# ihh/dnastore

Hardware: NVIDIA B200
Metric: viterbi_dp_cells_per_sec (higher is better)
Workload: dtype f64

## Files before the change

### dnastore_b200/csrc/viterbi_fill_batch.cu

```cuda
#include <cuda_runtime.h>

#include <cstdint>

#include "viterbi_batch.h"
#include "viterbi_kernels.h"

namespace dnab {
namespace {

__device__ __forceinline__ uint32_t smemAddr(const void* p) { return (uint32_t)__cvta_generic_to_shared(p); }
__device__ __forceinline__ double negInf() { return __longlong_as_double(0xFFF0000000000000LL); }
__device__ __forceinline__ double dmax(double a, double b) { return (a < b) ? b : a; }

__device__ __forceinline__ double2 ldsRow(uint32_t a) {
  double2 v;
  asm volatile("ld.volatile.shared.v2.f64 {%0,%1}, [%2];" : "=d"(v.x), "=d"(v.y) : "r"(a));
  return v;
}
__device__ __forceinline__ void stsRow(uint32_t a, double s, double d) {
  asm volatile("st.volatile.shared.v2.f64 [%0], {%1,%2};" ::"r"(a), "d"(s), "d"(d) : "memory");
}
__device__ __forceinline__ double2 ldPub2(const double2* p) {
  double2 v;
  asm volatile("ld.relaxed.gpu.global.v2.f64 {%0,%1}, [%2];" : "=d"(v.x), "=d"(v.y) : "l"(p) : "memory");
  return v;
}
__device__ __forceinline__ void stPub2(double2* p, double s, double d) {
  asm volatile("st.relaxed.gpu.global.v2.f64 [%0], {%1,%2};" ::"l"(p), "d"(s), "d"(d) : "memory");
}
__device__ __forceinline__ void stRecord(uint8_t* p, uint32_t v) {
  asm volatile("st.global.cs.u8 [%0], %1;" ::"l"(p), "r"(v) : "memory");
}
__device__ __forceinline__ uint32_t ldVolatileGlobal32(const uint32_t* p) {
  uint32_t v;
  asm volatile("ld.relaxed.gpu.global.u32 %0, [%1];" : "=r"(v) : "l"(p) : "memory");
  return v;
}
__device__ __forceinline__ unsigned long long ldAcquire64(const unsigned long long* p) {
  unsigned long long v;
  asm volatile("ld.acquire.gpu.global.u64 %0, [%1];" : "=l"(v) : "l"(p) : "memory");
  return v;
}

enum : uint32_t { kCtlFlag = 0, kCtlWake = 4, kCtlDecision = 8, kCtlPending = 16, kCtlPhase = 17, kCtlLock = 18, kCtlSeen = 32 };
constexpr uint32_t kKeepRecord = 0x100u;
constexpr uint32_t kKeepRecordWide = 0x10000u;

__device__ __forceinline__ void fenceRelease() { asm volatile("fence.release.gpu;" ::: "memory"); }
__device__ __forceinline__ void stRecordEarly(uint8_t* p, uint32_t v) { asm volatile("st.global.u8 [%0], %1;" ::"l"(p), "r"(v) : "memory"); }
__device__ __forceinline__ unsigned long long policyEvictLast() {
  unsigned long long pol;
  asm volatile("createpolicy.fractional.L2::evict_last.b64 %0, 1.0;" : "=l"(pol));
  return pol;
}
__device__ __forceinline__ double ldCarried(const double* p, unsigned long long pol) {
  double v;
  asm volatile("ld.global.L2::cache_hint.f64 %0, [%1], %2;" : "=d"(v) : "l"(p), "l"(pol) : "memory");
  return v;
}
__device__ __forceinline__ void stCarried(double* p, double v, unsigned long long pol) {
  asm volatile("st.global.L2::cache_hint.f64 [%0], %1, %2;" ::"l"(p), "d"(v), "l"(pol) : "memory");
}
__device__ __forceinline__ void redAdd32(uint32_t* p, uint32_t v) {
  asm volatile("red.relaxed.gpu.global.add.u32 [%0], %1;" ::"l"(p), "r"(v) : "memory");
}
__device__ __forceinline__ void stRelaxed32(uint32_t* p, uint32_t v) {
  asm volatile("st.relaxed.gpu.global.u32 [%0], %1;" ::"l"(p), "r"(v) : "memory");
}

}

template <int W, int KMAX, bool kTeam, bool kDebug, bool kWide>
__global__ void __launch_bounds__(W * 32, 1)
    viterbiFillBatchKernel(const __grid_constant__ BatchTables tb, const __grid_constant__ BatchArgs args) {
  extern __shared__ __align__(16) unsigned char smem[];
  constexpr uint32_t nThreads = W * 32;
  const uint32_t tid = threadIdx.x, lane = tid & 31u, warp = tid >> 5, lane16 = lane * 16u;
  const uint32_t T = kTeam ? tb.T : 1u, M = tb.M, k = tb.k, Np = T * M, N = tb.nStates, K2 = k + 2;
  const uint32_t team = kTeam ? blockIdx.x / T : blockIdx.x, rank = kTeam ? blockIdx.x - team * T : 0u;
  const uint32_t nSlots = (M + W - 1) / W;
  const double NEG = negInf();
  const BatchLayout lay = makeBatchLayout(M, tb.maxIn, tb.maxOut, tb.nSyms, kTeam);
  auto wideCounts = [&](const uint4& h) { return __ldg(tb.wide + bhWideNo(h)); };
  auto nOutLocalOf = [&](const uint4& h) { return (kWide && bhWide(h)) ? (wideCounts(h).w & 0xFFFFu) : bhNOutLocal(h); };
  auto nOutOf = [&](const uint4& h) { return (kWide && bhWide(h)) ? (wideCounts(h).w >> 16) : bhNOut(h); };

  const uint32_t aSD = smemAddr(smem + lay.sd);
  uint32_t* maskCur = reinterpret_cast<uint32_t*>(smem + lay.maskA);
  uint32_t* maskNext = reinterpret_cast<uint32_t*>(smem + lay.maskB);
  uint32_t* remInS = reinterpret_cast<uint32_t*>(smem + lay.remIn);
  uint32_t* clsOffS = reinterpret_cast<uint32_t*>(smem + lay.cls);
  uint32_t* clsStS = clsOffS + kNotifyClasses + 1;
  uint4* hdrS = reinterpret_cast<uint4*>(smem + lay.hdr);
  uint2* hdr2S = reinterpret_cast<uint2*>(smem + lay.hdr2);
  uint2* inS = reinterpret_cast<uint2*>(smem + lay.inE);
  uint2* relS = reinterpret_cast<uint2*>(smem + lay.relE);
  uint32_t* outS = reinterpret_cast<uint32_t*>(smem + lay.outE);
  double* tsE = reinterpret_cast<double*>(smem + lay.tsE);
  double* subS = reinterpret_cast<double*>(smem + lay.sub);
  volatile uint32_t* ctl = reinterpret_cast<volatile uint32_t*>(smem + lay.ctl);

  {
    for (uint32_t i = tid; i < M; i += nThreads) {
      hdrS[i] = tb.hdr[rank * M + i];
      hdr2S[i] = tb.hdr2[rank * M + i];
      if (kTeam) {
        remInS[i] = tb.remoteIn[rank * M + i];
        clsStS[i] = tb.clsStates[rank * M + i];
      }
      maskCur[i] = 0;
      maskNext[i] = 0;
    }
    const uint32_t inBase = tb.rankInOff[rank], nIn = tb.rankInOff[rank + 1] - inBase;
    for (uint32_t i = tid; i < nIn; i += nThreads) {
      uint2 e = tb.inEdges[inBase + i];
      if (!beRemote(e)) e.x = aSD + (e.x - rank * M) * 512u;
      inS[i] = e;
      uint2 q = tb.relEdges[inBase + i];
      relS[i] = q;
    }
    __syncthreads();
    for (uint32_t i = tid; i < M; i += nThreads) {
      const uint2 h2 = hdr2S[i];
      uint32_t nLoc = (h2.y & 0xFFu) + ((h2.y >> 8) & 0xFFu);
      if (kWide && bhWide(hdrS[i])) {
        const uint32_t lc = wideCounts(hdrS[i]).y;
        nLoc = (lc & 0xFFFFu) + (lc >> 16);
      }
      for (uint32_t j = 0; j < nLoc; ++j) relS[h2.x + j].x = aSD + (relS[h2.x + j].x - rank * M) * 512u;
    }
    const uint32_t outBase = tb.rankOutOff[rank], nOut = tb.rankOutOff[rank + 1] - outBase;
    for (uint32_t i = tid; i < nOut; i += nThreads) outS[i] = tb.outEdges[outBase + i];
    for (uint32_t i = tid; i < tb.nSyms * 16; i += nThreads) tsE[i] = tb.tsE[i];
    if (tid < 16) subS[tid] = tb.sub[tid];
    if (tid < 64) ctl[tid] = 0;
    if (kTeam && tid <= kNotifyClasses) clsOffS[tid] = tb.clsOff[rank * (kNotifyClasses + 1) + tid];
  }
  __syncthreads();

  const uint32_t privKinds = 2 + k;
  double* const privT = args.priv + (size_t)team * Np * privKinds * 32 + lane;
  const unsigned long long polLast = policyEvictLast();
  double2* const sdPubT = args.sdPub + (size_t)team * 2 * Np * 32;
  uint32_t* const notifyT = args.teamState + (size_t)team * T * kNotifyClasses;
  uint32_t* const passiveT = args.teamPassive + (size_t)team * 2;
  uint32_t notifySeen = 0;
  unsigned long long* const bar = args.barrier + team;
  unsigned long long barTarget = 0;
  uint32_t col = 0;

  auto teamBarrier = [&]() {
    __syncthreads();
    if (!kTeam) return;
    barTarget += T;
    if (tid == 0) {
      fenceRelease();
      atomicAdd(bar, 1ull);
      while (ldAcquire64(bar) < barTarget) {
      }
    }
    __syncthreads();
  };

  unsigned long long dbgLevels = 0, dbgVisits = 0, dbgEdges = 0, dbgWakes = 0, dbgClosure = 0, dbgRecord = 0, dbgPassive = 0, dbgInit = 0, dbgBarrier = 0, dbgRelaxCyc = 0, dbgFlushCyc = 0;

  for (int64_t group = team; group < args.nGroups; group += args.nTeams) {
    const int64_t slotIdx = group * 32 + lane;
    int64_t r = -1;
    if (args.order)
      r = args.order[slotIdx];
    else if (args.readBase + slotIdx < args.nReads)
      r = args.readBase + slotIdx;
    const int32_t L = r >= 0 ? args.readLen[r] : -1;
    const uint8_t* seq = r >= 0 ? args.packed + args.byteOff[r] : nullptr;
    int32_t Lmax = L;
    for (int sh = 16; sh > 0; sh >>= 1) Lmax = max(Lmax, __shfl_xor_sync(0xFFFFFFFFu, Lmax, sh));
    uint8_t* const predG = args.pred + (size_t)group * (size_t)(args.maxLen + 1) * N * K2 * 32;
    uint8_t* const predWideG = kWide ? args.predWide + (size_t)group * (size_t)(args.maxLen + 1) * tb.nWide * 64 + lane : nullptr;
    unsigned long long win = 0;
    uint32_t xNext = 0;

    for (int32_t pos = 0; pos <= Lmax; ++pos) {
      const bool act = pos <= L;
      if (pos < L) {
        if ((pos & 31) == 0) win = *reinterpret_cast<const unsigned long long*>(seq + (size_t)(pos >> 5) * 8);
        xNext = (uint32_t)(win >> (2 * (pos & 31))) & 3u;
      }
      const uint32_t par = col & 1u;
      ++col;
      unsigned long long stamp = 0;
      if (kDebug) stamp = clock64();
      double2* const sdPubCol = sdPubT + (size_t)par * Np * 32;
      double2* const sdPubNext = sdPubT + (size_t)(par ^ 1u) * Np * 32;
      uint32_t* const passiveCol = passiveT + par;

#pragma unroll 4
      for (uint32_t sl = 0; sl < nSlots; ++sl) {
        const uint32_t d = sl * W + warp;
        if (d < M) {
          double s0;
          if (pos == 0) {
            const uint4 h = hdrS[d];
            s0 = (!bhPad(h) && (tb.local || (rank == tb.startRank && d == tb.startLocal))) ? 0.0 : NEG;
            if (kTeam && bhRemoteOut(h)) stPub2(sdPubCol + (size_t)(rank * M + d) * 32 + lane, s0, NEG);
          } else
            s0 = ldCarried(privT + (size_t)(rank * M + d) * privKinds * 32, polLast);
          stsRow(aSD + d * 512u + lane16, s0, NEG);
        }
      }
      if (tid < 8) ctl[tid] = 0;
      if (tid == 0) {
        ctl[kCtlPending] = 0u;
        ctl[kCtlPhase] = 0u;
      }
      if (kDebug) {
        const unsigned long long t = clock64();
        dbgInit += t - stamp;
        stamp = t;
      }
      teamBarrier();
      if (kTeam && rank == 0 && tid == 0) stRelaxed32(passiveT + (par ^ 1u), 0u);
      if (kDebug) {
        const unsigned long long t = clock64();
        dbgBarrier += t - stamp;
        stamp = t;
      }

      const bool asyncClosure = args.asyncClosure != 0;
      uint32_t* const idleS = const_cast<uint32_t*>(reinterpret_cast<volatile uint32_t*>(ctl) + kCtlPending);
      uint32_t* const lockS = const_cast<uint32_t*>(reinterpret_cast<volatile uint32_t*>(ctl) + kCtlLock);
      uint32_t remotePending = 0;
      auto relax = [&](uint32_t sl, uint32_t m, bool allIn) -> bool {
        const uint32_t d = sl * W + warp;
        const uint4 h = hdrS[d];
        const uint2 h2 = hdr2S[d];
        uint32_t nLE = h2.y & 0xFFu, nLN = (h2.y >> 8) & 0xFFu, nRE = (h2.y >> 16) & 0xFFu, nRN = h2.y >> 24;
        if (kWide && bhWide(h)) {
          const uint4 wc = wideCounts(h);
          nLE = wc.y & 0xFFFFu;
          nLN = wc.y >> 16;
          nRE = wc.z & 0xFFFFu;
          nRN = wc.z >> 16;
        }
        const uint32_t eLN = nLE + nLN, eRE = eLN + nRE, nIn = eRE + nRN;
        const uint2* const rel = relS + h2.x;
        const uint32_t aOwn = aSD + d * 512u + lane16;
        const double2 own = ldsRow(aOwn);
        double s = own.x, dd = own.y;
        const char* const scoreBase = reinterpret_cast<const char*>(tb.symScore);
        auto scoreOf = [&](const uint2& e) { return *reinterpret_cast<const double*>(scoreBase + e.y); };
        auto emitFrom = [&](const double2 v, const uint2& e) {
          dd = dmax(dd, dmax(v.y + tb.delExtend, v.x + tb.delOpen) + scoreOf(e));
          if (kDebug) ++dbgEdges;
        };
        auto nullFrom = [&](const double2 v, const uint2& e) {
          const double sc = scoreOf(e);
          dd = dmax(dd, v.y + sc);
          s = dmax(s, v.x + sc);
          if (kDebug) ++dbgEdges;
        };
        auto one = [&](uint32_t j) {
          const uint2 e = rel[j];
          if (j < eLN) {
            const double2 v = ldsRow(e.x + lane16);
            if (j < nLE)
              emitFrom(v, e);
            else
              nullFrom(v, e);
          } else if (kTeam) {
            const double2 v = ldPub2(sdPubCol + (size_t)e.x * 32 + lane);
            if (j < eRE)
              emitFrom(v, e);
            else
              nullFrom(v, e);
          }
        };
        if (allIn || nIn <= 4u) {
          uint32_t j = 0;
#pragma unroll 1
          for (; j < nLE; ++j) {
            const uint2 e = rel[j];
            emitFrom(ldsRow(e.x + lane16), e);
          }
#pragma unroll 1
          for (; j < eLN; ++j) {
            const uint2 e = rel[j];
            nullFrom(ldsRow(e.x + lane16), e);
          }
          if (kTeam) {
#pragma unroll 1
            for (; j < eRE; ++j) {
              const uint2 e = rel[j];
              emitFrom(ldPub2(sdPubCol + (size_t)e.x * 32 + lane), e);
            }
#pragma unroll 1
            for (; j < nIn; ++j) {
              const uint2 e = rel[j];
              nullFrom(ldPub2(sdPubCol + (size_t)e.x * 32 + lane), e);
            }
          }
        } else {
          while (m) {
            const uint32_t j = (uint32_t)__ffs((int)m) - 1u;
            m &= m - 1u;
            if (j == 31u)
              for (uint32_t jj = 31; jj < nIn; ++jj) one(jj);
            else
              one(j);
          }
        }
        s = dmax(s, dd + tb.delEnd);
        const bool grew = act && ((s > own.x) || (dd > own.y));
        if (!__any_sync(0xFFFFFFFFu, grew)) return false;
        stsRow(aOwn, s, dd);
        if (kTeam && bhRemoteOut(h)) {
          stPub2(sdPubCol + (size_t)(rank * M + d) * 32 + lane, s, dd);
          remotePending |= 1u << sl;
        }
        const uint32_t nLoc = nOutLocalOf(h), outOff = bhOutOff(h);
        uint32_t* const flagTo = asyncClosure ? maskCur : maskNext;
#pragma unroll 1
        for (uint32_t o = lane; o < nLoc; o += 32) {
          const uint32_t w = outS[outOff + o];
          atomicOr(flagTo + boLocal(w), 1u << boBit(w));
        }
        return true;
      };
      auto flushRemote = [&]() {
        if (!kTeam || !remotePending) return;
        uint32_t nNotes = 0;
        for (uint32_t rp = remotePending; rp; rp &= rp - 1u) {
          const uint4 h = hdrS[((uint32_t)__ffs((int)rp) - 1u) * W + warp];
          nNotes += nOutOf(h) - nOutLocalOf(h);
        }
        const bool eager = args.eagerNotify != 0;
        if (lane == 0) redAdd32(passiveCol, 0u - (eager ? 2u * nNotes : nNotes));
        if (eager) {
          __syncwarp();
          for (uint32_t rp = remotePending; rp; rp &= rp - 1u) {
            const uint4 h = hdrS[((uint32_t)__ffs((int)rp) - 1u) * W + warp];
            const uint32_t first = bhOutOff(h) + nOutLocalOf(h), last = bhOutOff(h) + nOutOf(h);
            for (uint32_t o = first + lane; o < last; o += 32) redAdd32(notifyT + outS[o], 1u);
          }
        }
        fenceRelease();
        __syncwarp();
        while (remotePending) {
          const uint32_t sl = (uint32_t)__ffs((int)remotePending) - 1u;
          remotePending &= remotePending - 1u;
          const uint4 h = hdrS[sl * W + warp];
          const uint32_t first = bhOutOff(h) + nOutLocalOf(h), last = bhOutOff(h) + nOutOf(h);
          for (uint32_t o = first + lane; o < last; o += 32) redAdd32(notifyT + outS[o], 1u);
        }
      };

      if (asyncClosure) {
        const uint32_t iMine = lane * W + warp;
        const bool mineValid = lane < nSlots && iMine < M;
        bool idle = false;
        for (uint32_t sl = 0; sl < nSlots; ++sl) {
          const uint32_t d = sl * W + warp;
          if (d >= M) break;
          if (lane == 0) maskCur[d] = 0u;
          __syncwarp();
          unsigned long long tr = 0;
          if (kDebug) tr = clock64();
          relax(sl, 0, true);
          if (kDebug) dbgRelaxCyc += clock64() - tr;
        }
        {
          unsigned long long tr = 0;
          if (kDebug) tr = clock64();
          flushRemote();
          if (kDebug) dbgFlushCyc += clock64() - tr;
        }
        for (;;) {
          uint32_t mym = 0;
          if (mineValid) mym = reinterpret_cast<volatile uint32_t*>(maskCur)[iMine];
          uint32_t work = __ballot_sync(0xFFFFFFFFu, mym != 0);
          if (work) {
            if (idle) {
              if (lane == 0) atomicSub(idleS, 1u);
              idle = false;
              __syncwarp();
            }
            if (mym) atomicAnd(maskCur + iMine, ~mym);
            while (work) {
              const uint32_t sl = (uint32_t)__ffs((int)work) - 1u;
              work &= work - 1u;
              const uint32_t m = __shfl_sync(0xFFFFFFFFu, mym, sl);
              if (kDebug) ++dbgVisits;
              unsigned long long tr = 0;
              if (kDebug) tr = clock64();
              relax(sl, m, false);
              if (kDebug) dbgRelaxCyc += clock64() - tr;
            }
            {
              unsigned long long tr = 0;
              if (kDebug) tr = clock64();
              flushRemote();
              if (kDebug) dbgFlushCyc += clock64() - tr;
            }
            continue;
          }
          if (!idle) {
            if (lane == 0) atomicAdd(idleS, 1u);
            idle = true;
          }
          if (ctl[kCtlPhase] != 0u) break;
          uint32_t mine = 0;
          if (lane == 0) mine = ctl[kCtlLock] == 0u && atomicCAS(lockS, 0u, 1u) == 0u;
          if (!__shfl_sync(0xFFFFFFFFu, mine, 0)) {
            if (args.idleNs) __nanosleep(args.idleNs);
            continue;
          }
          auto unlock = [&]() {
            __syncwarp();
            if (lane == 0) {
              __threadfence_block();
              atomicExch(lockS, 0u);
            }
          };
          if (ctl[kCtlPhase] != 0u) {
            unlock();
            break;
          }
          bool quiet = false;
          if (ctl[kCtlPending] == W) {
            bool any = false;
            for (uint32_t i = lane; i < M; i += 32) any |= reinterpret_cast<volatile uint32_t*>(maskCur)[i] != 0u;
            quiet = !__any_sync(0xFFFFFFFFu, any) && ctl[kCtlPending] == W;
          }
          uint32_t action = 0;
          uint32_t delta = 0;
          if (!kTeam) {
            if (quiet) action = 2;
          } else {
            uint32_t seen = ctl[kCtlSeen + lane];
            auto pollClasses = [&]() -> uint32_t {
              const uint32_t c = ldVolatileGlobal32(notifyT + rank * kNotifyClasses + lane);
              delta = c - seen;
              seen = c;
              return __any_sync(0xFFFFFFFFu, delta != 0u) ? __reduce_add_sync(0xFFFFFFFFu, delta) : 0u;
            };
            uint32_t tot = pollClasses();
            if (tot) {
              if (lane == 0) redAdd32(passiveCol, tot);
              action = 1;
            } else if (quiet) {
              unsigned long long t0 = 0;
              if (kDebug) t0 = clock64();
              if (lane == 0) redAdd32(passiveCol, 1u);
              for (;;) {
                tot = pollClasses();
                if (tot) {
                  if (lane == 0) redAdd32(passiveCol, tot - 1u);
                  action = 1;
                  break;
                }
                uint32_t p = lane == 0 ? ldVolatileGlobal32(passiveCol) : 0u;
                p = __shfl_sync(0xFFFFFFFFu, p, 0);
                if (p == T) {
                  action = 2;
                  break;
                }
              }
              if (kDebug) dbgPassive += clock64() - t0;
            }
            ctl[kCtlSeen + lane] = seen;
          }
          if (action == 2) {
            if (lane == 0) ctl[kCtlPhase] = 1u;
            unlock();
          } else if (action == 1) {
            if (kDebug) ++dbgWakes;
            if (lane == 0) atomicSub(idleS, 1u);
            idle = false;
            __syncwarp();
            for (uint32_t notified = __ballot_sync(0xFFFFFFFFu, delta != 0u); notified; notified &= notified - 1u) {
              const uint32_t c = (uint32_t)__ffs((int)notified) - 1u;
              for (uint32_t q = clsOffS[c] + lane; q < clsOffS[c + 1]; q += 32) {
                const uint32_t i = clsStS[q];
                atomicOr(maskCur + i, remInS[i]);
              }
            }
            unlock();
          } else {
            unlock();
            if (args.idleNs) __nanosleep(args.idleNs / 2);
          }
        }
        __syncthreads();
      } else
      {
        auto notifyTotal = [&]() -> uint32_t {
          uint32_t t = 0;
          for (uint32_t q = 0; q < kNotifyClasses; ++q) t += ldVolatileGlobal32(notifyT + rank * kNotifyClasses + q);
          return t;
        };
        uint32_t lvl = 0;
        bool activated = false;
        for (uint32_t sl = 0; sl < nSlots; ++sl)
          if (sl * W + warp < M) activated |= relax(sl, 0, true);
        flushRemote();
        for (;;) {
          if (activated && lane == 0) ctl[kCtlFlag + ((lvl + 1) & 3u)] = 1u;
          if (tid == 0) {
            ctl[kCtlFlag + ((lvl + 2) & 3u)] = 0u;
            ctl[kCtlWake + ((lvl + 2) & 3u)] = 0u;
          }
          __syncthreads();
          {
            uint32_t* t = maskCur;
            maskCur = maskNext;
            maskNext = t;
          }
          ++lvl;
          const bool haveLocal = ctl[kCtlFlag + (lvl & 3u)] != 0;
          bool wake = kTeam && ctl[kCtlWake + (lvl & 3u)] != 0;
          if (!haveLocal && !wake) {
            if (!kTeam) break;
            if (tid == 0) {
              unsigned long long t0 = 0;
              if (kDebug) t0 = clock64();
              uint32_t decision;
              redAdd32(passiveCol, 1u);
              for (;;) {
                const uint32_t c = notifyTotal();
                if (c != notifySeen) {
                  redAdd32(passiveCol, c - notifySeen - 1u);
                  notifySeen = c;
                  decision = 1;
                  break;
                }
                if (ldVolatileGlobal32(passiveCol) == T) {
                  decision = 2;
                  break;
                }
              }
              ctl[kCtlDecision] = decision;
              if (kDebug) dbgPassive += clock64() - t0;
            }
            __syncthreads();
            if (ctl[kCtlDecision] == 2u) break;
            wake = true;
          }
          if (kDebug && haveLocal) ++dbgLevels;
          if (kDebug && wake) ++dbgWakes;
          activated = false;
          uint32_t st = 0;
          if (kTeam && tid == 0) st = notifyTotal();
          const uint32_t iMine = lane * W + warp;
          uint32_t mym = 0;
          if (lane < nSlots && iMine < M) {
            if (haveLocal) {
              mym = maskCur[iMine];
              if (mym) maskCur[iMine] = 0;
            }
            if (wake) mym |= remInS[iMine];
          }
          uint32_t work = __ballot_sync(0xFFFFFFFFu, mym != 0);
          while (work) {
            const uint32_t sl = (uint32_t)__ffs((int)work) - 1u;
            work &= work - 1u;
            const uint32_t m = __shfl_sync(0xFFFFFFFFu, mym, sl);
            if (kDebug) ++dbgVisits;
            activated |= relax(sl, m, false);
          }
          flushRemote();
          if (kTeam && tid == 0 && st != notifySeen) {
            redAdd32(passiveCol, st - notifySeen);
            notifySeen = st;
            ctl[kCtlWake + ((lvl + 1) & 3u)] = 1u;
          }
        }
      }
      if (kDebug) {
        const unsigned long long t = clock64();
        dbgClosure += t - stamp;
        stamp = t;
      }

      {
        double bv = NEG;
        uint32_t bo = 0xFFFFFFFFu;
        double pfB = NEG, pfT[KMAX];
        auto fetch = [&](uint32_t sl) {
          const uint32_t d = sl * W + warp;
          if (d < M && pos > 0) {
            const double* row = privT + (size_t)(rank * M + d) * privKinds * 32;
            pfB = ldCarried(row + 32, polLast);
#pragma unroll
            for (uint32_t t = 0; t < (uint32_t)KMAX; ++t)
              if (t < k) pfT[t] = ldCarried(row + 64 + 32 * t, polLast);
          }
        };
#pragma unroll
        for (uint32_t t = 0; t < (uint32_t)KMAX; ++t) pfT[t] = NEG;
        fetch(0);
        for (uint32_t sl = 0; sl < nSlots; ++sl) {
          const uint32_t d = sl * W + warp;
          if (d >= M) break;
          const double curB = pfB;
          double curT[KMAX];
#pragma unroll
          for (uint32_t t = 0; t < (uint32_t)KMAX; ++t) curT[t] = pfT[t];
          if (sl + 1 < nSlots) fetch(sl + 1);
          const uint4 h = hdrS[d];
          if (bhPad(h)) continue;
          const bool wide = kWide && bhWide(h);
          uint32_t nE = bhNEmit(h), nIn = nE + bhNNull(h);
          if (wide) {
            const uint32_t c = wideCounts(h).x;
            nE = c & 0xFFFFu;
            nIn = nE + (c >> 16);
          }
          const uint32_t inOff = bhInOff(h), mdl = bhMdl(h), orig = h.w;
          constexpr uint32_t keep = kWide ? kKeepRecordWide : kKeepRecord;
          const uint32_t none = wide ? kWideNoPred : kNoPred;
          double* const row = privT + (size_t)(rank * M + d) * privKinds * 32;
          const double2 own = ldsRow(aSD + d * 512u + lane16);
          const double sH = own.x, dH = own.y;
          double best = pos > 0 ? curB : NEG, bestD = NEG, s0n = NEG, bEn = NEG;
          uint32_t idx = pos > 0 ? keep : none, idxD = none, idxEn = none;
          uint32_t j = 0;
#pragma unroll 1
          for (; j < nE; ++j) {
            const uint2 e = inS[inOff + j];
            const uint32_t sym = beSym(e);
            const double2 v = (kTeam && beRemote(e)) ? ldPub2(sdPubCol + (size_t)e.x * 32 + lane) : ldsRow(e.x + lane16);
            double c = v.y + tb.tsDext[sym];
            if (c > bestD) {
              bestD = c;
              idxD = 2 * j;
            }
            c = v.x + tb.tsDopen[sym];
            if (c > bestD) {
              bestD = c;
              idxD = 2 * j + 1;
            }
            const uint32_t b4 = beBase(e) * 4 + xNext;
            s0n = dmax(s0n, ((v.x + tb.symScore[sym]) + tb.noGap) + subS[b4]);
            c = v.x + tsE[sym * 16 + b4];
            if (c > bEn) {
              bEn = c;
              idxEn = j;
            }
          }
#pragma unroll 1
          for (; j < nIn; ++j) {
            const uint2 e = inS[inOff + j];
            const double2 v = (kTeam && beRemote(e)) ? ldPub2(sdPubCol + (size_t)e.x * 32 + lane) : ldsRow(e.x + lane16);
            const double sc = tb.symScore[beSym(e)];
            double c = v.x + sc;
            if (c > best) {
              best = c;
              idx = j;
            }
            c = v.y + sc;
            if (c > bestD) {
              bestD = c;
              idxD = nE + j;
            }
          }
          {
            const double c = dH + tb.delEnd;
            if (c > best) {
              best = c;
              idx = nIn;
            }
          }
          if (mdl > 0 && pos > 0) {
            const double parked = curT[0];
            if (parked > best) {
              best = parked;
              idx = nIn + 1;
            }
          }
          if (tb.local && pos == 0) {
            const double2 v0 = (kTeam && tb.startRank != rank)
                                   ? ldPub2(sdPubCol + (size_t)(tb.startRank * M + tb.startLocal) * 32 + lane)
                                   : ldsRow(aSD + tb.startLocal * 512u + lane16);
            if (v0.x + 0.0 > best) {
              best = v0.x + 0.0;
              idx = nIn + 2;
            }
          }
          uint8_t* const pr = predG + ((size_t)pos * N + orig) * K2 * 32 + lane;
          uint8_t* const prW = wide ? predWideG + ((size_t)pos * tb.nWide + bhWideNo(h)) * 64 : nullptr;
          if (act) {
            if (idx != keep) stRecord(pr, idx);
            stRecord(pr + 32, idxD);
            if (wide) {
              if (idx != keep) stRecord(prW, idx >> 8);
              stRecord(prW + 32, idxD >> 8);
            }
          }
          double tNow[KMAX];
#pragma unroll
          for (uint32_t t = 0; t < (uint32_t)KMAX; ++t) {
            tNow[t] = NEG;
            if (t < k) {
              uint32_t idxT = kNoPred;
              if (pos > 0 && t < mdl) {
                double shifted = NEG;
                if (t + 1 < (uint32_t)KMAX && t + 1 < mdl) shifted = curT[t + 1 < (uint32_t)KMAX ? t + 1 : 0];
                if (shifted > NEG) idxT = 0;
                if (sH + tb.tsT[t] > shifted) idxT = 1;
                tNow[t] = dmax(shifted, (sH + tb.tanDup) + tb.len[t]);
              }
              if (act) stRecord(pr + (2 + t) * 32, idxT);
            }
          }
          if (kDebug && args.cells && group == 0 && lane == 0 && act) {
            double* cell = args.cells + ((size_t)pos * N + orig) * K2;
            cell[0] = sH;
            cell[1] = dH;
#pragma unroll
            for (uint32_t t = 0; t < (uint32_t)KMAX; ++t)
              if (t < k) cell[2 + t] = tNow[t];
          }
          if (mdl > 0) {
#pragma unroll
            for (uint32_t t = 0; t < (uint32_t)KMAX; ++t)
              if (t < mdl) {
                const double v = tNow[t] + subS[bhCtx(h, t) * 4 + xNext];
                if (t == 0) s0n = dmax(s0n, v);
                stCarried(row + 64 + 32 * t, v, polLast);
              }
          }
          stCarried(row, s0n, polLast);
          stCarried(row + 32, bEn, polLast);
          if (pos < L) {
            stRecordEarly(pr + (size_t)N * K2 * 32, idxEn);
            if (wide) stRecordEarly(prW + (size_t)tb.nWide * 64, idxEn >> 8);
          }
          if (kTeam && bhRemoteOut(h)) stPub2(sdPubNext + (size_t)(rank * M + d) * 32 + lane, s0n, NEG);
          if (!tb.local) {
            if (rank == tb.endRank && d == tb.endLocal && pos == L && r >= 0) args.loglike[r] = sH;
          } else if (sH > bv || (sH == bv && orig < bo)) {
            bv = sH;
            bo = orig;
          }
        }
        if (tb.local && pos == L) {
          args.partVal[((size_t)group * T * W + rank * W + warp) * 32 + lane] = bv;
          args.partOrig[((size_t)group * T * W + rank * W + warp) * 32 + lane] = bo;
        }
      }
      __syncthreads();
      if (kDebug) dbgRecord += clock64() - stamp;
    }
  }
  if (kDebug && args.dbg && lane == 0 && rank == 0) {
    if (warp == 0) atomicAdd(&args.dbg[1], dbgLevels);
    atomicAdd(&args.dbg[2], dbgVisits);
    atomicAdd(&args.dbg[3], dbgEdges);
    if (warp == 0) atomicAdd(&args.dbg[4], dbgClosure);
    if (warp == 0) atomicAdd(&args.dbg[5], dbgRecord);
    atomicAdd(&args.dbg[6], dbgWakes);
    atomicAdd(&args.dbg[7], dbgPassive);
    if (warp == 0) atomicAdd(&args.dbg[8], dbgInit);
    if (warp == 0) atomicAdd(&args.dbg[9], dbgBarrier);
    atomicAdd(&args.dbg[10], dbgRelaxCyc);
    atomicAdd(&args.dbg[11], dbgFlushCyc);
  }
}

__global__ void viterbiTracebackBatchKernel(const BatchTraceTables tb, const BatchTraceArgs args) {
  const int64_t slot = (int64_t)blockIdx.x * blockDim.x + threadIdx.x;
  if (slot >= args.nSlots) return;
  int64_t read = -1;
  if (args.order)
    read = args.order[slot];
  else if (args.readBase + slot < args.nReads)
    read = args.readBase + slot;
  if (read < 0) return;
  const int64_t group = slot >> 5;
  const uint32_t lane = (uint32_t)(slot & 31);
  const uint32_t N = tb.nStates, k = tb.k, K2 = k + 2;
  const int32_t L = args.readLen[read];
  const double NEG = negInf();

  uint32_t state;
  double ll;
  if (!tb.local) {
    state = N - 1;
    ll = args.loglike[read];
  } else {
    double bv = NEG;
    uint32_t bo = 0xFFFFFFFFu;
    for (uint32_t r = 0; r < tb.T; ++r) {
      const double v = args.partVal[((size_t)group * tb.T + r) * 32 + lane];
      const uint32_t o = args.partOrig[((size_t)group * tb.T + r) * 32 + lane];
      if (o == 0xFFFFFFFFu) continue;
      if (v > bv || (v == bv && o < bo)) {
        bv = v;
        bo = o;
      }
    }
    state = bo == 0xFFFFFFFFu ? 0u : bo;
    ll = bv;
    args.loglike[read] = ll;
  }

  char* out = args.decoded + (size_t)read * args.decodedStride;
  int32_t* path = args.path ? args.path + (size_t)read * 3 * args.pathStride : nullptr;
  int32_t nOut = 0, nPath = 0;
  int32_t status = DNAB_READ_OK_;
  if (!(ll > NEG)) {
    args.decodedLen[read] = 0;
    args.status[read] = DNAB_READ_NO_DECODING_;
    if (args.pathLen) args.pathLen[read] = 0;
    return;
  }
  const uint8_t* predG = args.pred + (size_t)group * (size_t)(args.maxLen + 1) * N * K2 * 32 + lane;
  const uint8_t* predWideG = args.predWide + (size_t)group * (size_t)(args.maxLen + 1) * tb.nWide * 64 + lane;
  int32_t pos = L;
  uint32_t mut = 0;
  const int32_t cap = args.decodedStride;
  while (pos >= 0 && state != 0) {
    if (path) {
      if (nPath < args.pathStride) {
        path[3 * nPath] = (int32_t)state;
        path[3 * nPath + 1] = pos;
        path[3 * nPath + 2] = (int32_t)mut;
      } else
        status = DNAB_READ_OVERFLOW_;
    }
    ++nPath;
    uint32_t p = predG[(((size_t)pos * N + state) * K2 + mut) * 32];
    uint32_t none = kNoPred;
    if (tb.wideOf && mut < 2) {
      const uint32_t wn = tb.wideOf[state];
      if (wn != 0xFFFFFFFFu) {
        p |= (uint32_t)predWideG[(((size_t)pos * tb.nWide + wn) * 2 + mut) * 32] << 8;
        none = kWideNoPred;
      }
    }
    if (p == none) {
      status = DNAB_READ_TRACEBACK_FAILED_;
      break;
    }
    const uint32_t e0 = tb.emitOff[state], nE = tb.emitOff[state + 1] - e0;
    const uint32_t n0 = tb.nullOff[state], nIn = nE + (tb.nullOff[state + 1] - n0);
    uint32_t sym = 0;
    if (mut == 0) {
      if (p < nE) {
        sym = tb.emitSym[e0 + p];
        state = tb.emitSrc[e0 + p];
        --pos;
      } else if (p < nIn) {
        sym = tb.nullSym[n0 + (p - nE)];
        state = tb.nullSrc[n0 + (p - nE)];
      } else if (p == nIn) {
        mut = 1;
      } else if (p == nIn + 1) {
        mut = 2;
        --pos;
      } else {
        state = 0;
      }
    } else if (mut == 1) {
      if (p < 2 * nE) {
        sym = tb.emitSym[e0 + (p >> 1)];
        state = tb.emitSrc[e0 + (p >> 1)];
        mut = (p & 1) ? 0 : 1;
      } else {
        sym = tb.nullSym[n0 + (p - 2 * nE)];
        state = tb.nullSrc[n0 + (p - 2 * nE)];
      }
    } else {
      if (p == 0) {
        mut += 1;
        --pos;
      } else
        mut = 0;
    }
    if (sym) {
      if (nOut < cap)
        out[cap - 1 - nOut] = (char)tb.symChar[sym];
      else
        status = DNAB_READ_OVERFLOW_;
      ++nOut;
    }
  }
  const int32_t kept = nOut < cap ? nOut : cap;
  for (int32_t i = 0; i < kept; ++i) out[i] = out[cap - kept + i];
  args.decodedLen[read] = kept;
  args.status[read] = status;
  if (args.pathLen) args.pathLen[read] = nPath;
}

typedef void (*BatchKernelPtr)(const BatchTables, const BatchArgs);
template <int W, int KMAX, bool kWide>
static BatchKernelPtr pickBatchKernelWK(bool team, bool debug) {
  if (debug) return team ? viterbiFillBatchKernel<W, KMAX, true, true, kWide> : viterbiFillBatchKernel<W, KMAX, false, true, kWide>;
  return team ? viterbiFillBatchKernel<W, KMAX, true, false, kWide> : viterbiFillBatchKernel<W, KMAX, false, false, kWide>;
}
static uint32_t batchWarps(uint32_t warps) { return warps > 24 ? 32u : warps > 16 ? 24u : 16u; }
template <bool kWide>
static BatchKernelPtr pickBatchKernelW(const BatchTables& tb, uint32_t warps, bool debug) {
  const bool team = tb.T > 1;
  const uint32_t w = batchWarps(warps);
  if (w == 32) return tb.k <= 2 ? pickBatchKernelWK<32, 2, kWide>(team, debug) : pickBatchKernelWK<32, kMaxK, kWide>(team, debug);
  if (w == 24) return tb.k <= 2 ? pickBatchKernelWK<24, 2, kWide>(team, debug) : pickBatchKernelWK<24, kMaxK, kWide>(team, debug);
  return tb.k <= 2 ? pickBatchKernelWK<16, 2, kWide>(team, debug) : pickBatchKernelWK<16, kMaxK, kWide>(team, debug);
}
static BatchKernelPtr pickBatchKernel(const BatchTables& tb, uint32_t warps, bool debug) {
  return tb.nWide ? pickBatchKernelW<true>(tb, warps, debug) : pickBatchKernelW<false>(tb, warps, debug);
}

cudaError_t queryBatchTeams(const BatchTables& tb, uint32_t warps, uint32_t smemBytes, int* ctasPerSm) {
  BatchKernelPtr kern = pickBatchKernel(tb, warps, false);
  cudaError_t err = cudaFuncSetAttribute(kern, cudaFuncAttributeMaxDynamicSharedMemorySize, (int)smemBytes);
  if (err != cudaSuccess) return err;
  return cudaOccupancyMaxActiveBlocksPerMultiprocessor(ctasPerSm, kern, (int)(batchWarps(warps) * 32), smemBytes);
}

cudaError_t launchFillBatch(const BatchTables& tb, const BatchArgs& args, uint32_t warps, uint32_t smemBytes,
                            cudaStream_t stream, size_t persistBytes) {
  const bool debug = args.dbg != nullptr || args.cells != nullptr;
  BatchKernelPtr kern = pickBatchKernel(tb, warps, debug);
  cudaError_t err = cudaFuncSetAttribute(kern, cudaFuncAttributeMaxDynamicSharedMemorySize, (int)smemBytes);
  if (err != cudaSuccess) return err;
  cudaLaunchConfig_t cfg{};
  cfg.gridDim = dim3(args.nTeams * tb.T);
  cfg.blockDim = dim3(batchWarps(warps) * 32);
  cfg.dynamicSmemBytes = smemBytes;
  cfg.stream = stream;
  cudaLaunchAttribute attr[2];
  unsigned nAttr = 0;
  if (tb.T > 1) {
    attr[nAttr].id = cudaLaunchAttributeCooperative;
    attr[nAttr].val.cooperative = 1;
    ++nAttr;
  }
  if (persistBytes) {
    attr[nAttr].id = cudaLaunchAttributeAccessPolicyWindow;
    attr[nAttr].val.accessPolicyWindow.base_ptr = args.priv;
    attr[nAttr].val.accessPolicyWindow.num_bytes = persistBytes;
    attr[nAttr].val.accessPolicyWindow.hitRatio = 1.0f;
    attr[nAttr].val.accessPolicyWindow.hitProp = cudaAccessPropertyPersisting;
    attr[nAttr].val.accessPolicyWindow.missProp = cudaAccessPropertyStreaming;
    ++nAttr;
  }
  cfg.attrs = attr;
  cfg.numAttrs = nAttr;
  return cudaLaunchKernelEx(&cfg, kern, tb, args);
}

cudaError_t launchTracebackBatch(const BatchTraceTables& tb, const BatchTraceArgs& args, cudaStream_t stream) {
  const int threads = 64;
  const int blocks = (int)((args.nSlots + threads - 1) / threads);
  viterbiTracebackBatchKernel<<<blocks, threads, 0, stream>>>(tb, args);
  return cudaGetLastError();
}

}
```

Measured before the change: 50.64 billion.

## Batch edge gathers in closure relax and prefetch next slot's predecessor rows

The closure relax step now handles incoming edges in groups of four. It loads all edge descriptors, scores and source rows before doing any max updates, so the load latencies overlap instead of being serialized. The final recurrence pass software-pipelines the first four incoming edges and their source rows for the next slot while the current slot computes. This adds register pressure and branchy bookkeeping for the mask and tail handling. The prefetch may also read shared or published rows before later relaxations update them, which needs care around ordering.

```diff
diff --git a/dnastore_b200/csrc/viterbi_fill_batch.cu b/dnastore_b200/csrc/viterbi_fill_batch.cu
--- a/dnastore_b200/csrc/viterbi_fill_batch.cu
+++ b/dnastore_b200/csrc/viterbi_fill_batch.cu
@@ -45,6 +45,7 @@
 enum : uint32_t { kCtlFlag = 0, kCtlWake = 4, kCtlDecision = 8, kCtlPending = 16, kCtlPhase = 17, kCtlLock = 18, kCtlSeen = 32 };
 constexpr uint32_t kKeepRecord = 0x100u;
 constexpr uint32_t kKeepRecordWide = 0x10000u;
+constexpr uint32_t kGather = 4;
 
 __device__ __forceinline__ void fenceRelease() { asm volatile("fence.release.gpu;" ::: "memory"); }
 __device__ __forceinline__ void stRecordEarly(uint8_t* p, uint32_t v) { asm volatile("st.global.u8 [%0], %1;" ::"l"(p), "r"(v) : "memory"); }
@@ -248,65 +249,66 @@
         const double2 own = ldsRow(aOwn);
         double s = own.x, dd = own.y;
         const char* const scoreBase = reinterpret_cast<const char*>(tb.symScore);
-        auto scoreOf = [&](const uint2& e) { return *reinterpret_cast<const double*>(scoreBase + e.y); };
-        auto emitFrom = [&](const double2 v, const uint2& e) {
-          dd = dmax(dd, dmax(v.y + tb.delExtend, v.x + tb.delOpen) + scoreOf(e));
+        auto emitFrom = [&](const double2 v, const double sc) {
+          dd = dmax(dd, dmax(v.y + tb.delExtend, v.x + tb.delOpen) + sc);
           if (kDebug) ++dbgEdges;
         };
-        auto nullFrom = [&](const double2 v, const uint2& e) {
-          const double sc = scoreOf(e);
+        auto nullFrom = [&](const double2 v, const double sc) {
           dd = dmax(dd, v.y + sc);
           s = dmax(s, v.x + sc);
           if (kDebug) ++dbgEdges;
         };
-        auto one = [&](uint32_t j) {
-          const uint2 e = rel[j];
-          if (j < eLN) {
-            const double2 v = ldsRow(e.x + lane16);
-            if (j < nLE)
-              emitFrom(v, e);
-            else
-              nullFrom(v, e);
-          } else if (kTeam) {
-            const double2 v = ldPub2(sdPubCol + (size_t)e.x * 32 + lane);
-            if (j < eRE)
-              emitFrom(v, e);
-            else
-              nullFrom(v, e);
-          }
+        auto gather = [&](const uint32_t(&js)[kGather], uint32_t n) {
+          uint2 e[kGather];
+          double sc[kGather];
+          double2 v[kGather];
+#pragma unroll
+          for (uint32_t i = 0; i < kGather; ++i) {
+            e[i] = make_uint2(0u, 0u);
+            sc[i] = 0.0;
+            v[i] = make_double2(0.0, 0.0);
+            if (i < n) e[i] = rel[js[i]];
+          }
+#pragma unroll
+          for (uint32_t i = 0; i < kGather; ++i)
+            if (i < n) {
+              sc[i] = *reinterpret_cast<const double*>(scoreBase + e[i].y);
+              v[i] = (!kTeam || js[i] < eLN) ? ldsRow(e[i].x + lane16) : ldPub2(sdPubCol + (size_t)e[i].x * 32 + lane);
+            }
+#pragma unroll
+          for (uint32_t i = 0; i < kGather; ++i)
+            if (i < n) {
+              if (js[i] < nLE || (kTeam && js[i] >= eLN && js[i] < eRE))
+                emitFrom(v[i], sc[i]);
+              else
+                nullFrom(v[i], sc[i]);
+            }
         };
-        if (allIn || nIn <= 4u) {
-          uint32_t j = 0;
-#pragma unroll 1
-          for (; j < nLE; ++j) {
-            const uint2 e = rel[j];
-            emitFrom(ldsRow(e.x + lane16), e);
-          }
-#pragma unroll 1
-          for (; j < eLN; ++j) {
-            const uint2 e = rel[j];
-            nullFrom(ldsRow(e.x + lane16), e);
-          }
-          if (kTeam) {
-#pragma unroll 1
-            for (; j < eRE; ++j) {
-              const uint2 e = rel[j];
-              emitFrom(ldPub2(sdPubCol + (size_t)e.x * 32 + lane), e);
-            }
-#pragma unroll 1
-            for (; j < nIn; ++j) {
-              const uint2 e = rel[j];
-              nullFrom(ldPub2(sdPubCol + (size_t)e.x * 32 + lane), e);
-            }
-          }
+        if (nIn <= kGather) {
+          uint32_t all[kGather];
+#pragma unroll
+          for (uint32_t i = 0; i < kGather; ++i) all[i] = i;
+          gather(all, nIn);
         } else {
-          while (m) {
-            const uint32_t j = (uint32_t)__ffs((int)m) - 1u;
-            m &= m - 1u;
-            if (j == 31u)
-              for (uint32_t jj = 31; jj < nIn; ++jj) one(jj);
-            else
-              one(j);
+          uint32_t mm = allIn ? (nIn >= 32u ? 0xFFFFFFFFu : (1u << nIn) - 1u) : m, tail = 31;
+          while (mm) {
+            uint32_t js[kGather], n = 0;
+#pragma unroll
+            for (uint32_t i = 0; i < kGather; ++i) {
+              js[i] = 0;
+              if (mm) {
+                const uint32_t j = (uint32_t)__ffs((int)mm) - 1u;
+                if (j < 31u) {
+                  js[i] = j;
+                  mm &= mm - 1u;
+                } else {
+                  js[i] = tail++;
+                  if (tail >= nIn) mm = 0;
+                }
+                n = i + 1;
+              }
+            }
+            gather(js, n);
           }
         }
         s = dmax(s, dd + tb.delEnd);
@@ -585,19 +587,51 @@
         double bv = NEG;
         uint32_t bo = 0xFFFFFFFFu;
         double pfB = NEG, pfT[KMAX];
+        uint32_t pfIn = 0;
+        uint2 pfE[kGather];
+        double2 pfV[kGather];
+#pragma unroll
+        for (uint32_t i = 0; i < kGather; ++i) {
+          pfE[i] = make_uint2(0u, 0u);
+          pfV[i] = make_double2(NEG, NEG);
+        }
+        auto srcRow = [&](const uint2& e) {
+          return (kTeam && beRemote(e)) ? ldPub2(sdPubCol + (size_t)e.x * 32 + lane) : ldsRow(e.x + lane16);
+        };
+        auto inCounts = [&](const uint4& h, uint32_t& nE, uint32_t& nIn) {
+          nE = bhNEmit(h);
+          nIn = nE + bhNNull(h);
+          if (kWide && bhWide(h)) {
+            const uint32_t c = wideCounts(h).x;
+            nE = c & 0xFFFFu;
+            nIn = nE + (c >> 16);
+          }
+        };
         auto fetch = [&](uint32_t sl) {
           const uint32_t d = sl * W + warp;
-          if (d < M && pos > 0) {
-            const double* row = privT + (size_t)(rank * M + d) * privKinds * 32;
-            pfB = ldCarried(row + 32, polLast);
-#pragma unroll
-            for (uint32_t t = 0; t < (uint32_t)KMAX; ++t)
-              if (t < k) pfT[t] = ldCarried(row + 64 + 32 * t, polLast);
+          pfIn = 0;
+          if (d < M) {
+            if (pos > 0) {
+              const double* row = privT + (size_t)(rank * M + d) * privKinds * 32;
+              pfB = ldCarried(row + 32, polLast);
+#pragma unroll
+              for (uint32_t t = 0; t < (uint32_t)KMAX; ++t)
+                if (t < k) pfT[t] = ldCarried(row + 64 + 32 * t, polLast);
+            }
+            const uint4 h = hdrS[d];
+            uint32_t nE;
+            inCounts(h, nE, pfIn);
+#pragma unroll
+            for (uint32_t i = 0; i < kGather; ++i)
+              if (i < pfIn) pfE[i] = inS[bhInOff(h) + i];
           }
         };
 #pragma unroll
         for (uint32_t t = 0; t < (uint32_t)KMAX; ++t) pfT[t] = NEG;
         fetch(0);
+#pragma unroll
+        for (uint32_t i = 0; i < kGather; ++i)
+          if (i < pfIn) pfV[i] = srcRow(pfE[i]);
         for (uint32_t sl = 0; sl < nSlots; ++sl) {
           const uint32_t d = sl * W + warp;
           if (d >= M) break;
@@ -605,16 +639,27 @@
           double curT[KMAX];
 #pragma unroll
           for (uint32_t t = 0; t < (uint32_t)KMAX; ++t) curT[t] = pfT[t];
-          if (sl + 1 < nSlots) fetch(sl + 1);
+          uint2 curE[kGather];
+          double2 curV[kGather];
+#pragma unroll
+          for (uint32_t i = 0; i < kGather; ++i) {
+            curE[i] = pfE[i];
+            curV[i] = pfV[i];
+          }
+          if (sl + 1 < nSlots)
+            fetch(sl + 1);
+          else
+            pfIn = 0;
           const uint4 h = hdrS[d];
-          if (bhPad(h)) continue;
+          if (bhPad(h)) {
+#pragma unroll
+            for (uint32_t i = 0; i < kGather; ++i)
+              if (i < pfIn) pfV[i] = srcRow(pfE[i]);
+            continue;
+          }
           const bool wide = kWide && bhWide(h);
-          uint32_t nE = bhNEmit(h), nIn = nE + bhNNull(h);
-          if (wide) {
-            const uint32_t c = wideCounts(h).x;
-            nE = c & 0xFFFFu;
-            nIn = nE + (c >> 16);
-          }
+          uint32_t nE, nIn;
+          inCounts(h, nE, nIn);
           const uint32_t inOff = bhInOff(h), mdl = bhMdl(h), orig = h.w;
           constexpr uint32_t keep = kWide ? kKeepRecordWide : kKeepRecord;
           const uint32_t none = wide ? kWideNoPred : kNoPred;
@@ -623,12 +668,8 @@
           const double sH = own.x, dH = own.y;
           double best = pos > 0 ? curB : NEG, bestD = NEG, s0n = NEG, bEn = NEG;
           uint32_t idx = pos > 0 ? keep : none, idxD = none, idxEn = none;
-          uint32_t j = 0;
-#pragma unroll 1
-          for (; j < nE; ++j) {
-            const uint2 e = inS[inOff + j];
+          auto emitCand = [&](const uint2& e, const double2& v, uint32_t j) {
             const uint32_t sym = beSym(e);
-            const double2 v = (kTeam && beRemote(e)) ? ldPub2(sdPubCol + (size_t)e.x * 32 + lane) : ldsRow(e.x + lane16);
             double c = v.y + tb.tsDext[sym];
             if (c > bestD) {
               bestD = c;
@@ -646,11 +687,8 @@
               bEn = c;
               idxEn = j;
             }
-          }
-#pragma unroll 1
-          for (; j < nIn; ++j) {
-            const uint2 e = inS[inOff + j];
-            const double2 v = (kTeam && beRemote(e)) ? ldPub2(sdPubCol + (size_t)e.x * 32 + lane) : ldsRow(e.x + lane16);
+          };
+          auto nullCand = [&](const uint2& e, const double2& v, uint32_t j) {
             const double sc = tb.symScore[beSym(e)];
             double c = v.x + sc;
             if (c > best) {
@@ -661,6 +699,27 @@
             if (c > bestD) {
               bestD = c;
               idxD = nE + j;
+            }
+          };
+#pragma unroll
+          for (uint32_t i = 0; i < kGather; ++i) {
+            if (i < nE)
+              emitCand(curE[i], curV[i], i);
+            else if (i < nIn)
+              nullCand(curE[i], curV[i], i);
+            if (i < pfIn) pfV[i] = srcRow(pfE[i]);
+          }
+          if (nIn > kGather) {
+            uint32_t j = kGather;
+#pragma unroll 1
+            for (; j < nE; ++j) {
+              const uint2 e = inS[inOff + j];
+              emitCand(e, srcRow(e), j);
+            }
+#pragma unroll 1
+            for (; j < nIn; ++j) {
+              const uint2 e = inS[inOff + j];
+              nullCand(e, srcRow(e), j);
             }
           }
           {
```

Result: slower. 37.63 billion, median of 6 (-25.7%).
